# google-deepmind/mujoco_warp

Hardware: AMD Instinct MI355X
Metric: env-steps/sec (nworld x steps/s) for humanoid.xml at 8192 worlds, 1/2/4/8 GPUs (higher is better)
Workload: dtype f32; 1 GPU; humanoid.xml, nworld=8192 per GPU, CG solver, Euler, pyramidal, nconmax=24, njmax=64, key 0 + Halton/OU control noise (std 0.01, rate 0.1); nworld_per_gpu=8192, nworld_total=8192, parallelism=worlds sharded over 1 GPU(s), no data-path collective

## Files before the change

### include/mjhip.h

```cpp
#ifndef MJHIP_H
#define MJHIP_H

#ifdef __cplusplus
extern "C" {
#endif

#define MJH_OK 0
#define MJH_E_ARG -1
#define MJH_E_UNSUPPORTED -2
#define MJH_E_LAUNCH -3

#define MJH_STAGE_KINEMATICS 0
#define MJH_STAGE_COM_POS 1
#define MJH_STAGE_CRB 2
#define MJH_STAGE_FACTOR_M 3
#define MJH_STAGE_COLLISION 4
#define MJH_STAGE_MAKE_CONSTRAINT 5
#define MJH_STAGE_TRANSMISSION 6
#define MJH_STAGE_COM_VEL 7
#define MJH_STAGE_PASSIVE 8
#define MJH_STAGE_RNE 9
#define MJH_STAGE_FWD_VELOCITY 10
#define MJH_STAGE_FWD_ACTUATION 11
#define MJH_STAGE_FWD_ACCELERATION 12
// ... 209 lines not shown
  float* actuator_length; float* actuator_moment;
  float* actuator_velocity; float* cvel; float* cdof_dot;
  float* qfrc_spring; float* qfrc_damper; float* qfrc_gravcomp; float* qfrc_passive; float* qfrc_bias;
  float* cacc; float* cfrc_int; float* cfrc_ext;
  float* act_dot; float* actuator_force; float* qfrc_actuator; float* qfrc_smooth; float* qacc_smooth;
  float* qacc; float* qfrc_constraint; float* efc_Ma;
  int* solver_niter; int* ne; int* nf; int* nl; int* nefc; int* overflow;
  int* nacon; int* ncollision;
  float* contact_dist; float* contact_pos; float* contact_frame; float* contact_includemargin;
  float* contact_friction; float* contact_solref; float* contact_solreffriction; float* contact_solimp;
  int* contact_dim; int* contact_geom; int* contact_efc_address; int* contact_worldid; int* contact_type;
  int* contact_geomcollisionid;
  int* efc_type; int* efc_id; int* efc_state;
  float* efc_J; float* efc_pos; float* efc_margin; float* efc_D; float* efc_vel; float* efc_aref;
  float* efc_frictionloss; float* efc_force;
  int* ws_ncon;
  int* ws_conadr;
  int* ws_ncollision;
  float* ws_ccd;
  int* ws_tree_rowadr;
  int* ws_tree_rowmap;
  int* ws_isl_dofadr;
  int* ws_isl_dofmap;
  int* ws_isl_dofinv;
  int* ws_nisland;
  int* ws_isl_flags;
  int* ws_isl_list;
  int* ws_isl_count;
  int* ws_separable;
  float* sensordata;
  float* subtree_linvel; float* subtree_angmom;
  float* energy;
  int* tree_asleep;
  int* tree_awake;
  int* body_awake;
  int* body_awake_ind;
  int* dof_awake_ind;
  int* ntree_awake; int* nbody_awake; int* nv_awake;
  int* tree_island;
  int* nisland;
  float* ws_iacc;
  float* ws_pgsB;
  float* ws_sleep_J;
  float* ws_sleep_warm;
  int* ws_sleep_flag;
  int sleep_pass;
  int nvmax;
  int* ws_efc_con;
  int* ws_order;
  int* eq_active;
  float* ws_rk;
  float* history;
  float* ws_ctrl_delayed;
  float* ws_contact;
} MjhData;

int mjh_stage(const MjhModel* m, const MjhData* d, int stage, void* stream);

int mjh_step(const MjhModel* m, const MjhData* d, void* stream);
int mjh_forward(const MjhModel* m, const MjhData* d, void* stream);

int mjh_solve_m(const MjhModel* m, const MjhData* d, float* x, const float* y, void* stream);
int mjh_mul_m(const MjhModel* m, const MjhData* d, float* res, const float* vec, void* stream);
int mjh_qld_dense(const MjhModel* m, const MjhData* d, float* qld_dense, int stride, void* stream);
int mjh_contact_force(const MjhModel* m, const MjhData* d, const int* contact_ids, int n, int to_world_frame, float* force, void* stream);
int mjh_jac(const MjhModel* m, const MjhData* d, float* jacp, float* jacr, const float* point, const int* body, void* stream);
int mjh_rays(const MjhModel* m, const MjhData* d, const float* pnt, const float* vec, int pnt_nworld, int nray, const float* geomgroup,
             int flg_static, const int* bodyexclude, float* dist, int* geomid, float* normal, void* stream);
int mjh_efc_j_sparse(const MjhModel* m, const MjhData* d, int njmax_nnz, int* rownnz, int* rowadr, int* colind, float* values, void* stream);

#define MJH_SET_CONST_FIXED 1
#define MJH_SET_CONST_0 2
int mjh_set_const(const MjhModel* m, int nbatch, float* body_subtreemass, float* dof_invweight0, float* body_invweight0, float* stat_meaninertia, int what,
                  void* stream);

typedef struct MjhRender {
  int nworld;
  int ncam;
  int npixel;
  int ntile;
  int groupmask;
  const int* cam_bodyid;
  const float* cam_pos;
  const float* cam_quat;
  const int* cam_res;
  const int* cam_exclude;
  const int* depth_adr;
  const int* seg_adr;
  const int* tile;
  const float* ray;
  float* depth;
  int* seg;
  float* normal;
  float* cam_xpos;
  float* cam_xmat;
} MjhRender;
int mjh_render(const MjhModel* m, const MjhData* d, const MjhRender* rc, void* stream);
int mjh_camera_rays(const MjhModel* m, const MjhData* d, const MjhRender* rc, float* pnt, float* vec, void* stream);

int mjh_ctrl_noise(const MjhModel* m, const MjhData* d, const float* ctrl_center, int step, float noise_std,
                   float noise_rate, void* stream);

int mjh_history_read(const MjhModel* m, const MjhData* d, int is_sensor, int id, const float* time, int interp, float* result, int result_stride,
                     void* stream);
int mjh_history_init(const MjhModel* m, const MjhData* d, int is_sensor, int id, const float* times, const float* values, int values_stride,
                     const float* phase, void* stream);
// ... 24 lines not shown
```

### mujoco_warp_amd/csrc/host.hpp

```cpp
#pragma once
#include <hip/hip_runtime.h>

#include <algorithm>
#include <cstdio>
#include <cstdlib>
#include <cstring>
#include <mutex>
#include <type_traits>
#include <vector>

#include "../../include/mjhip.h"
#include "dev_common.hpp"

int mjh_fail(int code, const char* fmt, const char* a = "");
#define fail mjh_fail
#define HIPCHK(expr)                                                      \
  do {                                                                    \
    hipError_t e_ = (expr);                                               \
    if (e_ != hipSuccess) return fail(MJH_E_LAUNCH, #expr ": %s", hipGetErrorString(e_)); \
  } while (0)

static const int kLdsPerCU = 160 * 1024;

const char* mjh_knob(const char* name);
// ... 24 lines not shown
  }
}
template <typename F>
static inline int dispatch_nv4_64(int nv4, F&& f) {
  if (nv4 <= 9) return f(std::integral_constant<int, 9>{});
  if (nv4 <= 10) return f(std::integral_constant<int, 10>{});
  if (nv4 <= 12) return f(std::integral_constant<int, 12>{});
  if (nv4 <= 14) return f(std::integral_constant<int, 14>{});
  return f(std::integral_constant<int, 16>{});
}

#ifdef MJH_PHASE_CLOCK
#define MJH_DEFINE_PHASE_TICKS                                                                                                      \
  extern "C" __attribute__((visibility("default"))) int mjh_debug_phase_ticks(unsigned long long* out, int reset) {               \
    if (out) HIPCHK(hipMemcpyFromSymbol(out, HIP_SYMBOL(g_phase_ticks), sizeof(unsigned long long) * 64 * 8 * 16));                 \
    if (reset) {                                                                                                                    \
      static unsigned long long zeros[64 * 8 * 16] = {0};                                                                           \
      HIPCHK(hipMemcpyToSymbol(HIP_SYMBOL(g_phase_ticks), zeros, sizeof(zeros)));                                                   \
    }                                                                                                                               \
    return MJH_OK;                                                                                                                  \
  }
#else
#define MJH_DEFINE_PHASE_TICKS
#endif

int pick_block(size_t shared_bytes, size_t per_world_bytes, int G, size_t* lds_out, bool prefer_small_arg = false);

template <typename K>
static hipError_t set_lds(K kernel, size_t bytes) {
  if (bytes <= 64 * 1024) return hipSuccess;
  static std::mutex mu;
  static std::vector<std::pair<const void*, size_t>> done;
  const void* f = reinterpret_cast<const void*>(kernel);
  std::lock_guard<std::mutex> lock(mu);
  for (auto& p : done)
    if (p.first == f && p.second >= bytes) return hipSuccess;
  hipError_t e = hipFuncSetAttribute(f, hipFuncAttributeMaxDynamicSharedMemorySize, (int)bytes);
  if (e == hipSuccess) done.emplace_back(f, bytes);
  return e;
}

template <typename K>
static void debug_occupancy(const char* name, K kernel, int grid, int threads, size_t lds) {
  if (!KNOB_ONCE_FLAG("MJH_DEBUG_OCC")) return;
  int nb = -1;
  (void)hipOccupancyMaxActiveBlocksPerMultiprocessor(&nb, kernel, threads, lds);
  fprintf(stderr, "%-22s grid %5d x %3d threads, LDS %6zu B: %2d workgroups per CU = %4.1f wavefronts per SIMD, %.2f rounds on 256 CUs\n", name, grid,
          threads, lds, nb, nb * (threads / 64) / 4.0, nb > 0 ? grid / (256.0 * nb) : 0.0);
}

int launch_solve_32_cg(const MjhModel* m, const MjhData* d, int nr, bool with_factor, int fuse_euler, hipStream_t s, int lo, int hi);
int launch_solve_32_newton_ell_r1(const MjhModel* m, const MjhData* d, bool with_factor, int fuse_euler, hipStream_t s, int lo, int hi);
int launch_solve_cgw(const MjhModel* m, const MjhData* d, bool with_factor, int fuse_euler, hipStream_t s, int lo, int hi);
int launch_solve_32_cg_deferred(const MjhModel* m, const MjhData* d, int fuse_euler, hipStream_t s);
int launch_solve_cgp(const MjhModel* m, const MjhData* d, bool with_factor, int fuse_euler, hipStream_t s);
int launch_solve_32_newton(const MjhModel* m, const MjhData* d, int nr, bool with_factor, int fuse_euler, hipStream_t s, int lo, int hi);
int launch_solve_newton_mfma(const MjhModel* m, const MjhData* d, bool with_factor, int fuse_euler, hipStream_t s);
int launch_solve_64_cg(const MjhModel* m, const MjhData* d, int nr, bool with_factor, int fuse_euler, hipStream_t s, int lo, int hi);
int launch_solve_64_newton(const MjhModel* m, const MjhData* d, int nr, bool with_factor, int fuse_euler, hipStream_t s, int lo, int hi);
int launch_solve_32_cg_ell(const MjhModel* m, const MjhData* d, int nr, bool with_factor, int fuse_euler, hipStream_t s, int lo, int hi);
int launch_solve_32_newton_ell(const MjhModel* m, const MjhData* d, int nr, bool with_factor, int fuse_euler, hipStream_t s, int lo, int hi);
int launch_solve_64_cg_ell(const MjhModel* m, const MjhData* d, int nr, bool with_factor, int fuse_euler, hipStream_t s, int lo, int hi);
int launch_solve_64_newton_ell(const MjhModel* m, const MjhData* d, int nr, bool with_factor, int fuse_euler, hipStream_t s, int lo, int hi);
int launch_solve_tree_cg(const MjhModel* m, const MjhData* d, hipStream_t s, hipStream_t sr, hipStream_t sr2, hipStream_t sr3);
int launch_solve_tree_newton(const MjhModel* m, const MjhData* d, hipStream_t s, hipStream_t sr, hipStream_t sr2, hipStream_t sr3);
int launch_solve_tree_cg_ell(const MjhModel* m, const MjhData* d, hipStream_t s, hipStream_t sr, hipStream_t sr2, hipStream_t sr3);
int launch_solve_tree_newton_ell(const MjhModel* m, const MjhData* d, hipStream_t s, hipStream_t sr, hipStream_t sr2, hipStream_t sr3);
int launch_pgs(const MjhModel* m, const MjhData* d, hipStream_t s);
int launch_pgs_big(const MjhModel* m, const MjhData* d, hipStream_t s);
int launch_solve_big(const MjhModel* m, const MjhData* d, hipStream_t s, int nefc_lo = -1);
int launch_render(const MjhModel* m, const MjhData* d, const MjhRender* rc, hipStream_t s);
int launch_camera_rays(const MjhModel* m, const MjhData* d, const MjhRender* rc, float* pnt, float* vec, hipStream_t s);
int launch_sensor_contact(const MjhModel* m, const MjhData* d, hipStream_t s);
int launch_sensor_collision(const MjhModel* m, const MjhData* d, hipStream_t s);
int launch_transmission(const MjhModel* m, const MjhData* d, hipStream_t s);
int launch_vel_trn(const MjhModel* m, const MjhData* d, int first, int last, bool lanes64, hipStream_t s);
int launch_history_ctrl(const MjhModel* m, const MjhData* d, int insert, hipStream_t s);
int launch_history_sensor(const MjhModel* m, const MjhData* d, int stage, int insert, hipStream_t s);
```

### mujoco_warp_amd/csrc/mjhip.hip

```cpp
#include "host.hpp"

#include "contact_rec.hpp"
#ifdef MJH_CON_WINDOW
#undef CON_WINDOW
#define CON_WINDOW MJH_CON_WINDOW
#endif
#ifndef MJH_MID_WAVES
#define MJH_MID_WAVES 4
#endif

#include "collide.hpp"
#include "constraint.hpp"
#include "dev_common.hpp"
#include "integrate.hpp"
#include "implicit.hpp"
#include "sensor.hpp"
#include "sleep.hpp"
#include "smooth.hpp"
#include "support.hpp"

static thread_local char g_err[512] = "";
int mjh_fail(int code, const char* fmt, const char* a) {
  snprintf(g_err, sizeof(g_err), fmt, a);
  return code;
// ... 434 lines not shown
    const int inl_force = KNOB_ONCE_INT("MJH_NEWTON_RIDERS", -1);
    const bool inl = step && !instrumented && (inl_force >= 0 ? inl_force != 0 : m->nv <= 16) && plan_family(m, d, p.ell, 0) == FAM_NEWTON_MFMA;
    const bool side = p.newton && m->nv <= KNOB_ONCE_INT("MJH_SIDE_NV", 32) && !instrumented && !inl && side_ok && !KNOB_ONCE_FLAG("MJH_NO_SIDE");
    p.riders = inl || (m->solver == SOL_CG && m->nv <= 64) ? RIDE_SOLVER : side ? RIDE_SIDE : RIDE_INTEGRATOR;
    const bool fusable = step && m->na == 0 && p.riders != RIDE_INTEGRATOR && m->nv <= 64 &&
                         m->nsensor_acc == 0 &&
                         d->njmax <= 192;
    p.fuse_euler = !fusable ? 0
                   : (m->integrator == INT_EULER && (m->disableflags & (DSBL_EULERDAMP | DSBL_DAMPER)) != 0) ? 1
                   : (m->integrator == INT_IMPLICITFAST && !KNOB_ONCE_FLAG("MJH_NO_FUSE_IMPLICITFAST") && !m->act_velfeedback) ? 2 : 0;
  }
  p.family = plan_family(m, d, p.ell, p.fuse_euler);
  p.r1 = p.family == FAM_NEWTON32_ELL && d->njmax > 32 && KNOB_ONCE_INT("MJH_SOLVE_R1", 1) != 0;
  return p;
}
static int launch_solve_any(const MjhModel* m, const MjhData* d, const StepPlan& p, const Run& run) {
  const hipStream_t s = run.s;
  const int fe = p.fuse_euler, all = 0x7fffffff;
  const bool with_factor = p.riders == RIDE_SOLVER;
  const int top = d->njmax > 192 ? 192 : all;
  switch (p.family) {
    case FAM_UNSUPPORTED: return solve_supported(m, d);
    case FAM_PGS: return launch_pgs(m, d, s);
    case FAM_PGS_BIG: return launch_pgs_big(m, d, s);
    case FAM_BIG: return launch_solve_big(m, d, s);
    case FAM_TREE_BIG: {
      hipLaunchKernelGGL(k_isl_clear, dim3(1), dim3(64), 0, s, *d);
      hipLaunchKernelGGL(k_tree_rows, dim3(d->nworld), dim3(64), sizeof(int) * (size_t)(2 * std::max(d->njmax, 1) + 2 * m->ntree), s, *m, *d);
      Streams* aux = side_streams(run);
      if (aux && aux->n < MJH_NAUX) aux = nullptr;
      int naux = 0;
      if (aux) {
        hipStreamCaptureStatus cst = hipStreamCaptureStatusNone;
        naux = (hipStreamIsCapturing(s, &cst) == hipSuccess && cst == hipStreamCaptureStatusActive) ? MJH_NAUX : MJH_NAUX_EAGER;
        const int cap = KNOB_ONCE_INT("MJH_NAUX", -1);
        if (cap >= 2 && cap <= MJH_NAUX) naux = cap;
      }
      hipStream_t s1 = aux ? aux->stream[0] : s, s2 = aux ? aux->stream[1] : s, s3 = naux > 2 ? aux->stream[2] : s1, s4 = naux > 3 ? aux->stream[3] : s1;
      if (aux) {
        HIPCHK(hipEventRecord(aux->fork, s));
        for (int k = 0; k < naux; ++k) HIPCHK(hipStreamWaitEvent(aux->stream[k], aux->fork, 0));
      }
      int rc = (p.newton ? (p.ell ? launch_solve_tree_newton_ell : launch_solve_tree_newton) : (p.ell ? launch_solve_tree_cg_ell : launch_solve_tree_cg))(m, d, s, s1, s3, s4);
      if (!rc) rc = launch_solve_big(m, d, s2);
      if (aux) {
        for (int k = 0; k < naux; ++k) {
          HIPCHK(hipEventRecord(aux->join[k], aux->stream[k]));
          HIPCHK(hipStreamWaitEvent(s, aux->join[k], 0));
        }
      }
      return rc;
    }
    case FAM_NEWTON_MFMA: return launch_solve_newton_mfma(m, d, with_factor, fe, s);
    case FAM_CGP: {
      if (int rc = launch_solve_cgp(m, d, with_factor, fe, s)) return rc;
      return launch_solve_32_cg_deferred(m, d, fe, s);
    }
    case FAM_CGW:
    case FAM_PAIR:
    case FAM_CG32_ELL:
    case FAM_NEWTON32:
    case FAM_NEWTON32_ELL: {
      auto s32 = p.ell ? (p.newton ? launch_solve_32_newton_ell : launch_solve_32_cg_ell) : (p.newton ? launch_solve_32_newton : launch_solve_32_cg);
      const bool wide = p.family == FAM_CGW;
      int lo2 = -1;
      if (p.r1) {
        if (int rc = launch_solve_32_newton_ell_r1(m, d, false, fe, s, -1, 32)) return rc;
        lo2 = 32;
      }
      if (d->njmax <= 64) return wide ? launch_solve_cgw(m, d, with_factor, fe, s, -1, all) : s32(m, d, 2, with_factor, fe, s, lo2, all);
      if (int rc = wide ? launch_solve_cgw(m, d, false, fe, s, -1, 64) : s32(m, d, 2, false, fe, s, lo2, 64)) return rc;
      if (int rc = s32(m, d, 6, with_factor, fe, s, 64, top)) return rc;
      return d->njmax > 192 ? launch_solve_big(m, d, s, 192) : MJH_OK;
    }
    case FAM_CG64:
    case FAM_CG64_ELL:
    case FAM_NEWTON64:
    case FAM_NEWTON64_ELL: {
      auto s64 = p.ell ? (p.newton ? launch_solve_64_newton_ell : launch_solve_64_cg_ell) : (p.newton ? launch_solve_64_newton : launch_solve_64_cg);
      if (d->njmax <= 64) return s64(m, d, 1, with_factor, fe, s, -1, all);
      if (d->njmax <= 128) return s64(m, d, 2, with_factor, fe, s, -1, all);
      if (int rc = s64(m, d, 2, with_factor, fe, s, -1, 128)) return rc;
      if (int rc = s64(m, d, 3, false, fe, s, 128, top)) return rc;
      return d->njmax > 192 ? launch_solve_big(m, d, s, 192) : MJH_OK;
    }
  }
  return fail(MJH_E_ARG, "launch_solve_any: unknown solver family");
}
static int launch_solve(const MjhModel* m, const MjhData* d, const Run& run) { return launch_solve_any(m, d, plan_step(m, d, MJH_STAGE_SOLVE, run.instr != nullptr), run); }
static const char* solver_kernel_name(const MjhModel* m, const MjhData* d) { return kFamilyName[plan_step(m, d, MJH_STAGE_STEP, false).family]; }
static int launch_integrate_plus(const MjhModel* m, const MjhData* d, int mode, bool integrate, bool with_factor, hipStream_t s) {
  constexpr int G = 32;
  const IntLayout lay = int_layout(m->nv, m->nC);
  const FacLayout fl = fac_layout(m->nv, m->nC);
  const size_t ms_bytes = sizeof(int) * mstruct_ints(m->nv, m->nC);
  size_t lds = std::max(ms_bytes + sizeof(float) * std::max(lay.total, fl.total) * (256 / G), (size_t)2048);
  if (lds > (size_t)kLdsPerCU) return fail(MJH_E_UNSUPPORTED, "k_integrate: does not fit in LDS");
  HIPCHK(set_lds(k_integrate_plus<G>, lds));
  const int nb = (d->nworld + 256 / G - 1) / (256 / G);
  const int nint = integrate ? nb : 0, npub = with_factor ? nb : 0, nfac = with_factor ? nb : 0;
  if (nint + npub + nfac == 0) return MJH_OK;
  if (integrate && mode == 2) TRY(launch_implicit(m, d, s));
  debug_occupancy("k_integrate_plus", k_integrate_plus<G>, nint + npub + nfac, 256, lds);
  hipLaunchKernelGGL(k_integrate_plus<G>, dim3(nint + npub + nfac), dim3(256), lds, s, *m, *d, mode, nint, npub);
  return MJH_OK;
}
static void apply_noise(const MjhModel* m, const MjhData* d, Run& run) {
  const NoiseArgs noise = run.noise;
  run.noise.n = 0;
  if (noise.n == 0) return;
// ... 484 lines not shown
```

### mujoco_warp_amd/csrc/solve_cg32.hip

```cpp
#include "solve_tu.hpp"

int launch_solve_32_cg(const MjhModel* m, const MjhData* d, int nr, bool with_factor, int fuse_euler, hipStream_t s, int lo, int hi) {
  switch (nr) {
    case 2: return launch_solve_32<2, false>(m, d, with_factor, fuse_euler, s, lo, hi);
    case 6: return launch_solve_32<6, false>(m, d, with_factor, fuse_euler, s, lo, hi);
    default: return fail(MJH_E_ARG, "k_solve: unsupported rows per lane");
  }
}

int launch_solve_32_cg_deferred(const MjhModel* m, const MjhData* d, int fuse_euler, hipStream_t s) {
  return dispatch_nv4_32((m->nv + 3) / 4, [&](auto NV4) { return launch_solve_deferred_t<NV4(), 2, false, 32>(m, d, fuse_euler, s); });
}

MJH_DEFINE_PHASE_TICKS
```

### mujoco_warp_amd/csrc/solve_cgp.hip

```cpp
#include "host.hpp"

#include "contact_rec.hpp"
#include "smooth.hpp"
#include "solver_cgp.hpp"

#ifndef CGP_WAVES
#define CGP_WAVES 3
#endif
#define CGP_MAXT (256 * CGP_WAVES)
template <int NV4>
__global__ void __launch_bounds__(CGP_MAXT) __attribute__((amdgpu_waves_per_eu(CGP_WAVES, CGP_WAVES))) k_solve_cgp_plus(MjhModel m, MjhData d, int nsolve, int nfac, int fuse_euler, int pool_rows) {
  extern __shared__ __attribute__((aligned(16))) float smem[];
  const int wpb = blockDim.x / 32;
  if ((int)blockIdx.x < nsolve) solve_cgp_body<NV4>(m, d, smem, (int)blockIdx.x * wpb, wpb, pool_rows, fuse_euler);
  else {
    const int bi = (int)blockIdx.x - nsolve;
    if (bi < nfac) factor_smooth_body<32>(m, d, 0, smem, Blk{bi * wpb, wpb, (int)blockDim.x});
    else publish_body<32>(d, 1, reinterpret_cast<int*>(smem), Blk{(bi - nfac) * wpb, wpb, (int)blockDim.x}, m.nexplicit ? m.pair_solreffriction : nullptr);
  }
}
template <int NV4>
static int launch_cgp_t(const MjhModel* m, const MjhData* d, bool with_factor, int fuse_euler, hipStream_t s) {
  int threads = 128;
  if (const char* e = knob_str("MJH_CGP_THREADS")) threads = std::min(CGP_MAXT, std::max(64, (atoi(e) / 64) * 64));
  size_t lds = ((size_t)kLdsPerCU / (256 * CGP_WAVES / threads)) & ~(size_t)1023;
  if (const char* e = knob_str("MJH_CGP_LDS")) lds = (size_t)atoi(e);
  const int wpb = threads / 32;
  const int pool_rows = cgp_pool_rows<NV4>(lds, wpb);
  if (pool_rows < cgp_min_rows<NV4>(fuse_euler)) return fail(MJH_E_UNSUPPORTED, "k_solve_cgp: pool too small");
  const FacLayout fl = fac_layout(m->nv, m->nC);
  if (with_factor) lds = std::max(lds, sizeof(int) * mstruct_ints(m->nv, m->nC) + sizeof(float) * fl.total * wpb);
  if (lds > (size_t)kLdsPerCU) return fail(MJH_E_UNSUPPORTED, "k_solve_cgp: the workgroup does not fit in LDS");
  HIPCHK(set_lds(k_solve_cgp_plus<NV4>, lds));
  const int nsolve = (d->nworld + wpb - 1) / wpb, nfac = with_factor ? nsolve : 0;
  debug_occupancy("k_solve_cgp_plus", k_solve_cgp_plus<NV4>, nsolve + 2 * nfac, threads, lds);
  hipLaunchKernelGGL(k_solve_cgp_plus<NV4>, dim3(nsolve + 2 * nfac), dim3(threads), lds, s, *m, *d, nsolve, nfac, fuse_euler, pool_rows);
  return MJH_OK;
}
int launch_solve_cgp(const MjhModel* m, const MjhData* d, bool with_factor, int fuse_euler, hipStream_t s) {
  return dispatch_nv4_32((m->nv + 3) / 4, [&](auto NV4) { return launch_cgp_t<NV4()>(m, d, with_factor, fuse_euler, s); });
}

MJH_DEFINE_PHASE_TICKS
```

### mujoco_warp_amd/csrc/solve_tu.hpp

```cpp
#pragma once
#include "host.hpp"

#include "contact_rec.hpp"
#include "smooth.hpp"
#include "solver.hpp"

#ifndef MJH_N64_WAVES
#define MJH_N64_WAVES 1
#endif

template <int NV4, int NR, bool NEWTON, int SG, bool ELL = false>
__global__ void __launch_bounds__(256) __attribute__((amdgpu_waves_per_eu((!NEWTON && !ELL && SG == 32 && NR == 2) ? 3 : ((NEWTON && SG == 64 && MJH_N64_WAVES > 1) ? MJH_N64_WAVES : 1), 8))) k_solve_plus(MjhModel m, MjhData d, int nsolve, int nfac, int nefc_lo, int nefc_hi, int fuse_euler, int rider_at) {
  extern __shared__ __attribute__((aligned(16))) float smem[];
  const int wpb = blockDim.x / SG;
  const int bx = (int)blockIdx.x, nrider = NEWTON ? 0 : 2 * nfac;
  const int sb = bx < rider_at ? bx : bx - nrider;
  if (bx < rider_at || bx >= rider_at + nrider) solve_body<NV4, NR, NEWTON, SG, ELL>(m, d, smem, Blk{sb * wpb, wpb, (int)blockDim.x}, nefc_lo, nefc_hi, fuse_euler);
  else if (!NEWTON) {
    const int wf = blockDim.x / 32, bi = bx - rider_at;
    if (bi < nfac) factor_smooth_body<32>(m, d, 0, smem, Blk{bi * wf, wf, (int)blockDim.x});
    else publish_body<32>(d, 1, reinterpret_cast<int*>(smem), Blk{(bi - nfac) * wf, wf, (int)blockDim.x}, m.nexplicit ? m.pair_solreffriction : nullptr);
  }
}
template <int NV4, int NR, bool NEWTON, int SG, bool ELL = false>
static int launch_solve_t(const MjhModel* m, const MjhData* d, bool with_factor, int fuse_euler, hipStream_t s, int nefc_lo, int nefc_hi) {
  const SolveLayout lay = solve_layout<NV4, NR, SG, NEWTON, ELL>(std::min(d->njmax, nefc_hi));
  const FacLayout fl = fac_layout(m->nv, m->nC);
  const size_t ms_bytes = sizeof(int) * mstruct_ints(m->nv, m->nC);
  size_t lds;
  int threads = pick_block(0, sizeof(float) * lay.total, SG, &lds, true);
  if (!threads) return fail(MJH_E_UNSUPPORTED, "k_solve: njmax x nv does not fit in LDS");
  if (const char* e = knob_str("MJH_SOLVE_THREADS")) {
    threads = std::max(atoi(e), SG);
    lds = sizeof(float) * lay.total * (threads / SG);
  }
  const int wpb = threads / SG, wf = threads / 32;
  with_factor = with_factor && !NEWTON;
  if (with_factor) lds = std::max(lds, ms_bytes + sizeof(float) * fl.total * wf);
  HIPCHK(set_lds((k_solve_plus<NV4, NR, NEWTON, SG, ELL>), lds));
  const int nsolve = (d->nworld + wpb - 1) / wpb, nfac = with_factor ? (d->nworld + wf - 1) / wf : 0;
  debug_occupancy(NEWTON ? "k_solve_plus<newton>" : "k_solve_plus<cg>", k_solve_plus<NV4, NR, NEWTON, SG, ELL>, nsolve + 2 * nfac, threads, lds);
  const int rider_pct = KNOB_ONCE_INT("MJH_RIDER_AT", 100);
  const int rider_at = std::min(nsolve, (int)((long long)nsolve * std::max(rider_pct, 0) / 100));
  hipLaunchKernelGGL((k_solve_plus<NV4, NR, NEWTON, SG, ELL>), dim3(nsolve + 2 * nfac), dim3(threads), lds, s, *m, *d, nsolve, nfac, nefc_lo, nefc_hi, fuse_euler, rider_at);
  return MJH_OK;
}
template <int NV4, int NR, bool NEWTON, int SG, bool ELL = false>
__global__ void __launch_bounds__(256) k_solve_deferred(MjhModel m, MjhData d, int fuse_euler) {
  extern __shared__ __attribute__((aligned(16))) float smem[];
  const int wpb = blockDim.x / SG;
  const int lig = threadIdx.x & (SG - 1), gid = (int)blockIdx.x * wpb + (int)threadIdx.x / SG;
  for (int c0 = gid * SG; c0 < d.nworld; c0 += (int)gridDim.x * wpb * SG) {
    unsigned long long todo = gballot<SG>(c0 + lig < d.nworld && d.solver_niter[c0 + lig] == -1);
    while (todo) {
      const int bq = __ffsll((long long)todo) - 1;
      todo &= todo - 1ull;
      solve_body<NV4, NR, NEWTON, SG, ELL>(m, d, smem, Blk{0, wpb, (int)blockDim.x}, -1, 0x7fffffff, fuse_euler, 0, 0x7fffffff, c0 + bq);
      gsync();
    }
  }
}
template <int NV4, int NR, bool NEWTON, int SG, bool ELL = false>
static int launch_solve_deferred_t(const MjhModel* m, const MjhData* d, int fuse_euler, hipStream_t s) {
  const SolveLayout lay = solve_layout<NV4, NR, SG, NEWTON, ELL>(d->njmax);
  size_t lds;
  const int threads = pick_block(0, sizeof(float) * lay.total, SG, &lds, true);
  if (!threads) return fail(MJH_E_UNSUPPORTED, "k_solve_deferred: njmax x nv does not fit in LDS");
  HIPCHK(set_lds((k_solve_deferred<NV4, NR, NEWTON, SG, ELL>), lds));
  const int wpb = threads / SG;
  hipLaunchKernelGGL((k_solve_deferred<NV4, NR, NEWTON, SG, ELL>), dim3(std::max(1, (d->nworld + wpb * SG - 1) / (wpb * SG))), dim3(threads), lds, s, *m, *d, fuse_euler);
  return MJH_OK;
}
template <int NR, bool NEWTON, bool ELL = false>
static int launch_solve_32(const MjhModel* m, const MjhData* d, bool wf, int fe, hipStream_t s, int lo, int hi) {
  return dispatch_nv4_32((m->nv + 3) / 4, [&](auto NV4) { return launch_solve_t<NV4(), NR, NEWTON, 32, ELL>(m, d, wf, fe, s, lo, hi); });
}
template <int NR, bool NEWTON, bool ELL = false>
static int launch_solve_64(const MjhModel* m, const MjhData* d, bool wf, int fe, hipStream_t s, int lo, int hi) {
  return dispatch_nv4_64((m->nv + 3) / 4, [&](auto NV4) { return launch_solve_t<NV4(), NR, NEWTON, 64, ELL>(m, d, wf, fe, s, lo, hi); });
}
```

### mujoco_warp_amd/csrc/solver.hpp

```cpp
#pragma once
#include "dev_common.hpp"
#include "smooth.hpp"

template <int G>
DEV float bcastg(float v, int k) {
  const int a = __builtin_amdgcn_readlane(__float_as_int(v), k);
  if (G == 64) return __int_as_float(a);
  const int b = __builtin_amdgcn_readlane(__float_as_int(v), k + 32);
  return __int_as_float((threadIdx.x & 32) ? b : a);
}
template <int G>
DEV float gsumg(float v) {
  v = dpp_add_f<0x111, 0xf, 0xf>(v);
  v = dpp_add_f<0x112, 0xf, 0xf>(v);
  v = dpp_add_f<0x114, 0xf, 0xf>(v);
  v = dpp_add_f<0x118, 0xf, 0xf>(v);
  v = dpp_add_f<0x142, 0xa, 0xf>(v);
  if (G == 64) {
    v = dpp_add_f<0x143, 0xc, 0xf>(v);
    return bcastg<64>(v, 63);
  }
  return __int_as_float(__builtin_amdgcn_ds_swizzle(__float_as_int(v), 0x3E0));
}
template <int G, int N>
// ... 589 lines not shown
    gsync();
    float P[4][4], Pi[4][4];
#pragma unroll
    for (int p = 0; p < 4; ++p) {
      const float4 v = *reinterpret_cast<const float4*>(pb + p * NVR + k);
      P[p][0] = v.x; P[p][1] = v.y; P[p][2] = v.z; P[p][3] = v.w;
#pragma unroll
      for (int e = 0; e < 4; ++e) Pi[p][e] = p == e ? 1.0f : 0.0f;
    }
#pragma unroll
    for (int j = 0; j < 4; ++j) {
      const float ip = 1.0f / P[j][j];
#pragma unroll
      for (int e = 0; e < 4; ++e) {
        P[j][e] *= ip;
        Pi[j][e] *= ip;
      }
#pragma unroll
      for (int r = 0; r < 4; ++r)
        if (r != j) {
          const float f = P[r][j];
#pragma unroll
          for (int e = 0; e < 4; ++e) {
            P[r][e] -= f * P[j][e];
            Pi[r][e] -= f * Pi[j][e];
          }
        }
    }
    const bool inb = q >= 0 && q < 4;
    float F[4];
#pragma unroll
    for (int p = 0; p < 4; ++p) {
      const float out = s[k] * Pi[0][p] + s[k + 1] * Pi[1][p] + s[k + 2] * Pi[2][p] + s[k + 3] * Pi[3][p];
      const float own = (q == p ? 1.0f : 0.0f) - (q == 0 ? Pi[0][p] : (q == 1 ? Pi[1][p] : (q == 2 ? Pi[2][p] : Pi[3][p])));
      F[p] = inb ? own : out;
    }
#pragma unroll
    for (int c4 = 0; c4 < NVR / 4; ++c4) {
      if (c4 == kb) continue;
      const float4 r0 = *reinterpret_cast<const float4*>(pb + 4 * c4), r1 = *reinterpret_cast<const float4*>(pb + NVR + 4 * c4),
                   r2 = *reinterpret_cast<const float4*>(pb + 2 * NVR + 4 * c4), r3 = *reinterpret_cast<const float4*>(pb + 3 * NVR + 4 * c4);
      s[4 * c4] -= F[0] * r0.x + F[1] * r1.x + F[2] * r2.x + F[3] * r3.x;
      s[4 * c4 + 1] -= F[0] * r0.y + F[1] * r1.y + F[2] * r2.y + F[3] * r3.y;
      s[4 * c4 + 2] -= F[0] * r0.z + F[1] * r1.z + F[2] * r2.z + F[3] * r3.z;
      s[4 * c4 + 3] -= F[0] * r0.w + F[1] * r1.w + F[2] * r2.w + F[3] * r3.w;
    }
#pragma unroll
    for (int e = 0; e < 4; ++e) s[k + e] = (q == e ? 1.0f : 0.0f) - F[e];
  }
}

template <int NV4, int NR, bool NEWTON, int G, bool ELL = false, bool TREE = false>
DEV void solve_body(const MjhModel& m, const MjhData& d, float* smem, const Blk& b, int nefc_lo = -1, int nefc_hi = 0x7fffffff,
                    int fuse_euler = 0, int nv_lo = 0, int nv_hi = 0x7fffffff, int w_direct = -1) {
  if ((int)threadIdx.x >= b.nthreads) return;
  constexpr int NVR = 4 * NV4;
  constexpr int JS = (NV4 & 1) ? NVR : NVR + 4;
  const int nv_all = m.nv, nC = m.nC, njmax = d.njmax, nvp = d.nv_pad;
  const SolveLayout lay = solve_layout<NV4, NR, G, NEWTON, ELL, TREE>(TREE ? njmax : min(njmax, nefc_hi));
  const int lig = threadIdx.x & (G - 1), gib = threadIdx.x / G;
  const int slot = b.w0 + gib;
  if (TREE && gib >= b.nw) return;
  if (w_direct < 0 && slot >= (TREE ? d.nworld * m.ntree : d.nworld)) return;
  const int w = TREE ? slot / m.ntree : (w_direct >= 0 ? w_direct : d.ws_order[slot]);
  const int tree = TREE ? slot - w * m.ntree : 0;
  if (TREE && (!d.ws_separable[w] || tree >= d.ws_nisland[w])) return;
  const int* dadr = TREE ? d.ws_isl_dofadr + (size_t)w * (m.ntree + 1) + tree : nullptr;
  const int nv = TREE ? dadr[1] - dadr[0] : nv_all;
  if (TREE && (nv <= nv_lo || nv > nv_hi)) return;
  const int* dmap = TREE ? d.ws_isl_dofmap + (size_t)w * nv_all + dadr[0] : nullptr;
  const int* dinv = TREE ? d.ws_isl_dofinv + (size_t)w * nv_all : nullptr;
  const int* rmap = TREE ? d.ws_tree_rowmap + (size_t)w * njmax + d.ws_tree_rowadr[(size_t)w * (m.ntree + 1) + tree] : nullptr;
  auto R = [&](int r) __attribute__((always_inline)) { return TREE ? rmap[r] : r; };
  float* S = smem + (size_t)gib * lay.total;
  float *Jl = S + lay.J, *eforce = S + lay.force, *eda = S + lay.da, *bsearch = S + lay.bsearch, *bgrad = S + lay.bgrad, *col = S + lay.col;
  constexpr int GR = G * NR;
  float *exu = S + lay.ex, *exv = exu + GR, *exq0 = exv + GR, *exq1 = exq0 + GR, *exq2 = exq1 + GR, *exs = exq2 + GR;
  float* econe = S + lay.cone;
  int* einfo = reinterpret_cast<int*>(S + lay.cone) + 6 * GR;

  const int nefc_all = TREE ? d.ws_tree_rowadr[(size_t)w * (m.ntree + 1) + tree + 1] - d.ws_tree_rowadr[(size_t)w * (m.ntree + 1) + tree]
                            : min(d.nefc[w], njmax);
  if (nefc_all <= nefc_lo || nefc_all > nefc_hi) return;
  const int nefc = min(nefc_all, G * NR);
  const int ne = TREE ? 0 : d.ne[w], nf = TREE ? 0 : d.nf[w];
  const size_t vo = TREE ? (size_t)w * nv_all + (lig < nv ? dmap[lig] : 0) - lig : (size_t)w * nv_all, eo = (size_t)w * njmax;
  float* flds = S + lay.fl;
  bool has_fl = nf > 0;
  if (TREE) {
    bool any = false;
    for (int r = lig; r < G * NR; r += G) {
      const bool fr = r < nefc && (d.efc_type[eo + rmap[r]] == CT_FRICTION_DOF || d.efc_type[eo + rmap[r]] == CT_FRICTION_TENDON);
      flds[r] = fr ? d.efc_frictionloss[eo + rmap[r]] : 0.0f;
      any |= fr;
    }
    has_fl = gballot<G>(any) != 0ull;
    gsync();
  }
  const float* floss = TREE ? flds : d.efc_frictionloss + eo;
  const bool active = lig < nv;
  const int ligr = lig < NVR ? lig : NVR - 1;

  PhaseClock pc(5, lig);
  float mrow[NVR];
  if (!TREE) {
    const float* Mg = d.M + (size_t)w * nC;
    const int nv4r = (nv_all + 3) >> 2;
    const int4* tab = reinterpret_cast<const int4*>(m.M_dense) + (size_t)(active ? lig : 0) * nv4r;
    int idx[NVR];
#pragma unroll
    for (int c4 = 0; c4 < NV4; ++c4) {
      const int4 t4 = c4 < nv4r ? tab[c4] : make_int4(-1, -1, -1, -1);
      idx[4 * c4] = t4.x; idx[4 * c4 + 1] = t4.y; idx[4 * c4 + 2] = t4.z; idx[4 * c4 + 3] = t4.w;
    }
#pragma unroll
    for (int c = 0; c < NVR; ++c) {
      const float v = Mg[idx[c] < 0 ? 0 : idx[c]];
      mrow[c] = active ? (idx[c] < 0 ? 0.0f : v) : (c == lig ? 1.0f : 0.0f);
    }
  } else {
    for (int idx = lig; idx < NVR * JS; idx += G) Jl[idx] = 0.0f;
    gsync();
    const float* Mg = d.M + (size_t)w * nC;
    for (int i = lig; i < nv; i += G) {
      const int gi = TREE ? dmap[i] : i;
      const int start = m.M_rowadr[gi], n = m.M_rownnz[gi];
      for (int a = 0; a < n; ++a) {
// ... 566 lines not shown
```

### mujoco_warp_amd/csrc/solver_cgp.hpp

```cpp
#pragma once
#include <type_traits>
#include "solver.hpp"
#include "solver_cgw.hpp"

#ifndef MJH_CGP_HOIST
#define MJH_CGP_HOIST 1
#endif
#define CGP_HEAD 32
#define CGP_WORLD 136
template <int NV4>
__host__ __device__ inline int cgp_pool_rows(size_t lds_bytes, int wpb) {
  constexpr int NVR = 4 * NV4, JS = (NV4 & 1) ? NVR : NVR + 4;
  const int words = (int)(lds_bytes / sizeof(float)) - CGP_HEAD - CGP_WORLD * wpb;
  return words <= 0 ? 0 : ((words / JS) & ~3);
}
template <int NV4>
__host__ __device__ inline int cgp_min_rows(int fuse_euler) {
  constexpr int NVR = 4 * NV4, JS = (NV4 & 1) ? NVR : NVR + 4;
  const int words = fuse_euler == 2 ? (6 * 32 + 12 * NV4 + 4 + 32) : (8 * NVR > 32 ? 8 * NVR : 32);
  return (((words + JS - 1) / JS) + 3) & ~3;
}

template <int CTRL>
DEV float qperm(float v) {
// ... 135 lines not shown
  {
    const float* Mg = d.M + (size_t)w * nC;
#pragma unroll
    for (int c = 0; c < NVR; ++c) {
      const float v = Mg[idx[c] < 0 ? 0 : idx[c]];
      mrow[c] = active ? (idx[c] < 0 ? 0.0f : v) : (c == lig ? 1.0f : 0.0f);
    }
  }
  const float fs = active ? d.qfrc_smooth[vo + lig] : 0.0f;
  const float qwarm = active ? d.qacc_warmstart[vo + lig] : 0.0f;

  int np = 0, nq = 0, need = 0;
  bool defer = false;
  if (valid) {
    npf = min(npf, nefc);
    bool is6[2];
#pragma unroll
    for (int k = 0; k < 2; ++k) {
      const int r = lig + G * k;
      is6[k] = r >= npf && r < nefc && ty[k] == CT_CONTACT_PYRAMIDAL;
    }
    const unsigned m0 = (unsigned)gballot<G>(is6[0]), m1 = (unsigned)gballot<G>(is6[1]);
    const int n60 = __popc(m0), n6 = n60 + __popc(m1);
    const unsigned below = (1u << lig) - 1u;
#pragma unroll
    for (int k = 0; k < 2; ++k) {
      const int r = lig + G * k;
      const int c6 = k == 0 ? __popc(m0 & below) : n60 + __popc(m1 & below);
      if (r < nefc && r < 64) slotR[is6[k] ? c6 : n6 + r - c6] = r;
      fbT[r] = 0.0f;
    }
    nq = n6 >> 2;
    np = nefc - n6;
    defer = nf > 0 || (n6 & 3) != 0 || nefc > 64;
    need = max((np + 3 * nq + 15) & ~15, cgp_min_rows<NV4>(fuse_euler));
  }
  if (lig == 0 && gib < CGP_HEAD) cnt[gib] = (valid && !defer) ? need : 0;
  __syncthreads();
  int base = 0;
  {
    int acc = 0;
    for (int j = 0; j < nwb; ++j) {
      const int c = cnt[j];
      const bool fits = acc + c <= pool_rows;
      if (j == gib) {
        base = acc;
        if (!fits) defer = true;
      }
      acc += fits ? c : 0;
    }
  }
  if (!valid) return;
  if (defer) {
    if (lig == 0) d.solver_niter[w] = -1;
    return;
  }
  float* Jl = pool + (size_t)base * JS;
  const int nb = np + 3 * nq, nb16 = (nb + 15) & ~15;

  PhaseClock pc(5, lig);
  pc.mark(0);
  const bool warm = !(m.disableflags & DSBL_WARMSTART);
  auto mul_row = [&](const float (&row)[NVR], BV x) __attribute__((always_inline)) {
    float s[2] = {0.0f, 0.0f};
    dpp_fence(x);
    fmac_seq<0, NVR, NA>(s, row, x.a);
    if constexpr (NBX > 0) fmac_seq<NA, NVR, NBX>(s, row, x.b);
    return active ? s[0] + s[1] : 0.0f;
  };
  float h[NVR];
  invert_rows_b4s<NVR, G>(mrow, h, Jl, lig);
  float qs = mul_row(h, bcast_prep(fs));
  {
    const float res = fs - mul_row(mrow, bcast_prep(qs));
    qs += mul_row(h, bcast_prep(active ? res : 0.0f));
  }
  if (active) d.qacc_smooth[vo + lig] = qs;
  float q = active ? (nefc > 0 && warm ? qwarm : qs) : 0.0f;
  pc.mark(1);
  float Ma = mul_row(mrow, bcast_prep(q));
  if (nefc == 0) {
    if (active) {
      d.qacc[vo + lig] = q;
      d.qfrc_constraint[vo + lig] = 0.0f;
      d.efc_Ma[vo + lig] = Ma;
    }
    if (lig == 0) d.solver_niter[w] = 0;
    if (fuse_euler) {
      float qi = q;
      gsync();
      if (fuse_euler == 2) qi = impfast_acc<NV4, G>(m, d, w, lig, active, mrow, Ma, Jl);
      euler_advance<G>(m, d, w, lig, active, qi, Jl + (fuse_euler == 2 ? 6 * G + 12 * NV4 + 4 : 0), q);
    }
    return;
  }

  float rD[NR], rja[NR], rjv[NR];
  int rkind[NR];
  int jro[NR];
  int fbo[NR];
  bool isq[NR];
  int rer[NR];
  const int qd = lig & 3;
#pragma unroll
  for (int k = 0; k < NR; ++k) {
    const int s = lig + G * k;
    const bool has = s < nefc;
// ... 269 lines not shown
```

### mujoco_warp_amd/types.py

```python

import dataclasses
import enum

import numpy as np

from .device import DeviceArray


class BroadphaseType(enum.IntEnum):
  NXN = 0
  SAP_TILE = 1
  SAP_SEGMENTED = 2


class BroadphaseFilter(enum.IntFlag):
  PLANE = 1 << 0
  SPHERE = 1 << 1
  AABB = 1 << 2
  OBB = 1 << 3


class OverflowType(enum.IntFlag):
  NEFC = 1 << 0
  NJMAX_NNZ = 1 << 1
# ... 617 lines not shown
  subtree_com: DeviceArray = _arr(('nworld', 'nbody', 3), "float32")
  cinert: DeviceArray = _arr(('nworld', 'nbody', 10), "float32")
  cdof: DeviceArray = _arr(('nworld', 'nv', 6), "float32")
  crb: DeviceArray = _arr(('nworld', 'nbody', 10), "float32")
  M: DeviceArray = _arr(('nworld', 'nC'), "float32")
  qLD: DeviceArray = _arr(('nworld', 'nC'), "float32")
  qLDiagInv: DeviceArray = _arr(('nworld', 'nv'), "float32")
  actuator_length: DeviceArray = _arr(('nworld', 'nu'), "float32")
  actuator_moment: DeviceArray = _arr_own(('nworld', 'nJmom'), "float32")
  moment_rownnz: DeviceArray = _arr(('nworld', 'nu'), "int32")
  moment_rowadr: DeviceArray = _arr(('nworld', 'nu'), "int32")
  moment_colind: DeviceArray = _arr_own(('nworld', 'nJmom'), "int32")
  actuator_velocity: DeviceArray = _arr(('nworld', 'nu'), "float32")
  cvel: DeviceArray = _arr(('nworld', 'nbody', 6), "float32")
  cdof_dot: DeviceArray = _arr(('nworld', 'nv', 6), "float32")
  qfrc_spring: DeviceArray = _arr(('nworld', 'nv'), "float32")
  qfrc_damper: DeviceArray = _arr(('nworld', 'nv'), "float32")
  qfrc_gravcomp: DeviceArray = _arr(('nworld', 'nv'), "float32")
  qfrc_passive: DeviceArray = _arr(('nworld', 'nv'), "float32")
  qfrc_bias: DeviceArray = _arr(('nworld', 'nv'), "float32")
  cacc: DeviceArray = _arr(('nworld', 'nbody', 6), "float32")
  cfrc_int: DeviceArray = _arr(('nworld', 'nbody', 6), "float32")
  act_dot: DeviceArray = _arr(('nworld', 'na'), "float32")
  actuator_force: DeviceArray = _arr(('nworld', 'nu'), "float32")
  qfrc_actuator: DeviceArray = _arr(('nworld', 'nv'), "float32")
  qfrc_smooth: DeviceArray = _arr(('nworld', 'nv'), "float32")
  qacc_smooth: DeviceArray = _arr(('nworld', 'nv'), "float32")
  qacc: DeviceArray = _arr(('nworld', 'nv'), "float32")
  qfrc_constraint: DeviceArray = _arr(('nworld', 'nv'), "float32")
  solver_niter: DeviceArray = _arr(('nworld',), "int32")
  ne: DeviceArray = _arr(('nworld',), "int32")
  nf: DeviceArray = _arr(('nworld',), "int32")
  nl: DeviceArray = _arr(('nworld',), "int32")
  nefc: DeviceArray = _arr(('nworld',), "int32")
  overflow: DeviceArray = _arr(('nworld',), "int32")
  nacon: DeviceArray = _arr((1,), "int32")
  ncollision: DeviceArray = _arr((1,), "int32")
  ws_ncon: DeviceArray = _arr(('nworld',), "int32")
  ws_conadr: DeviceArray = _arr(('nworld',), "int32")
  ws_ncollision: DeviceArray = _arr(('nworld',), "int32")
  ws_efc_con: DeviceArray = _arr(('nworld', 'njmax'), "int32")
  ws_tree_rowadr: DeviceArray = _arr(('nworld', 'ntreeadr'), "int32")
  ws_tree_rowmap: DeviceArray = _arr(('nworld', 'ntreerow'), "int32")
  ws_isl_dofadr: DeviceArray = _arr(('nworld', 'ntreeadr'), "int32")
  ws_isl_dofmap: DeviceArray = _arr(('nworld', 'ntreedof'), "int32")
  ws_isl_dofinv: DeviceArray = _arr(('nworld', 'ntreedof'), "int32")
  ws_nisland: DeviceArray = _arr(('nworld',), "int32")
  ws_isl_flags: DeviceArray = _arr(('nworld',), "int32")
  ws_isl_list: DeviceArray = _arr((3, 'ntreeworld'), "int32")
  ws_isl_count: DeviceArray = _arr((4,), "int32")
  ws_separable: DeviceArray = _arr(('nworld',), "int32")
  ws_ccd: DeviceArray = _arr(('nccdworld', 'nccdword', 32), "float32")
  ws_order: DeviceArray = _arr(('nworld',), "int32")
  sensordata: DeviceArray = _arr(('nworld', 'nsensordata'), "float32")
  energy: DeviceArray = _arr(('nworld', 2), "float32")
  subtree_linvel: DeviceArray = _arr(('nworld', 'nbody', 3), "float32")
  subtree_angmom: DeviceArray = _arr(('nworld', 'nbody', 3), "float32")
  cfrc_ext: DeviceArray = _arr(('nworld', 'nbody', 6), "float32")
  tree_asleep: DeviceArray = _arr(('nworld', 'ntree'), "int32")
  tree_awake: DeviceArray = _arr(('nworld', 'ntree'), "int32")
  body_awake: DeviceArray = _arr(('nworld', 'nbody'), "int32")
  body_awake_ind: DeviceArray = _arr(('nworld', 'nbody'), "int32")
  dof_awake_ind: DeviceArray = _arr(('nworld', 'nv'), "int32")
  ntree_awake: DeviceArray = _arr(('nworld',), "int32")
  nbody_awake: DeviceArray = _arr(('nworld',), "int32")
  nv_awake: DeviceArray = _arr(('nworld',), "int32")
  tree_island: DeviceArray = _arr(('nworld', 'ntree'), "int32")
  nisland: DeviceArray = _arr(('nworld',), "int32")
  ws_iacc: DeviceArray = _arr(('nimpworld', 'nv'), "float32")
  ws_pgsB: DeviceArray = _arr(('npgsworld', 'njmax_pad', 'nv_pad'), "float32")
  ws_sleep_J: DeviceArray = _arr(('nsleepworld', 'njmax_pad', 'nv_pad'), "float32")
  ws_sleep_warm: DeviceArray = _arr(('nsleepworld', 'nv'), "float32")
  ws_sleep_flag: DeviceArray = _arr(('nworld',), "int32")
  sleep_pass: int = 0
  nimpworld: int = 0
  npgsworld: int = 0
  nvmax: int = 0
  nsleepworld: int = 0
  eq_active: DeviceArray = _arr(('nworld', 'neq'), "int32")
  ws_rk: DeviceArray = _arr(('nworld', 'nq+3*nv+2*na'), "float32")
  ws_contact: DeviceArray = _arr(('nworld', 'concap', 32), "float32")
  history: DeviceArray = _arr_own(('nworld', 'nhistory'), "float32")
  ws_ctrl_delayed: DeviceArray = _arr(('nworld', 'nu'), "float32")
  nworld: int = 0
  nconmax: int = 0
  naconmax: int = 0
  njmax: int = 0
  njmax_pad: int = 0
  nv_pad: int = 0
  nmaxpyramid: int = 0
  nccdworld: int = 0
  nccdword: int = 0
  world_offset: int = 0
  concap: int = 0
  nccdhand: int = 0
  njmax_nnz: int = 0
```

Baseline: 27.87 million env-steps/s.

## Fold deferred CG fallback solve into last-finishing block of CGP kernel

Removes the separate k_solve_deferred launch after the CGP solver. Worlds whose constraint rows do not fit the LDS pool now increment a global counter; the last wave to finish, chosen by an atomic ticket, solves those deferred worlds inside the same kernel, reloading the kernel arguments from the kernarg segment. This saves a kernel launch and its full grid scan of solver_niter. In exchange, deferred worlds run serially in a single workgroup, the kernel's LDS request grows to the fallback layout size, and a new 8-byte control word must be allocated and zeroed.

```diff
diff --git a/include/mjhip.h b/include/mjhip.h
--- a/include/mjhip.h
+++ b/include/mjhip.h
@@ -285,6 +285,7 @@
   float* ws_rk;
   float* history;
   float* ws_ctrl_delayed;
+  int* ws_cgp_ctl;
   float* ws_contact;
 } MjhData;
 
diff --git a/mujoco_warp_amd/csrc/host.hpp b/mujoco_warp_amd/csrc/host.hpp
--- a/mujoco_warp_amd/csrc/host.hpp
+++ b/mujoco_warp_amd/csrc/host.hpp
@@ -100,7 +100,6 @@
 int launch_solve_32_cg(const MjhModel* m, const MjhData* d, int nr, bool with_factor, int fuse_euler, hipStream_t s, int lo, int hi);
 int launch_solve_32_newton_ell_r1(const MjhModel* m, const MjhData* d, bool with_factor, int fuse_euler, hipStream_t s, int lo, int hi);
 int launch_solve_cgw(const MjhModel* m, const MjhData* d, bool with_factor, int fuse_euler, hipStream_t s, int lo, int hi);
-int launch_solve_32_cg_deferred(const MjhModel* m, const MjhData* d, int fuse_euler, hipStream_t s);
 int launch_solve_cgp(const MjhModel* m, const MjhData* d, bool with_factor, int fuse_euler, hipStream_t s);
 int launch_solve_32_newton(const MjhModel* m, const MjhData* d, int nr, bool with_factor, int fuse_euler, hipStream_t s, int lo, int hi);
 int launch_solve_newton_mfma(const MjhModel* m, const MjhData* d, bool with_factor, int fuse_euler, hipStream_t s);
diff --git a/mujoco_warp_amd/csrc/mjhip.hip b/mujoco_warp_amd/csrc/mjhip.hip
--- a/mujoco_warp_amd/csrc/mjhip.hip
+++ b/mujoco_warp_amd/csrc/mjhip.hip
@@ -510,10 +510,7 @@
       return rc;
     }
     case FAM_NEWTON_MFMA: return launch_solve_newton_mfma(m, d, with_factor, fe, s);
-    case FAM_CGP: {
-      if (int rc = launch_solve_cgp(m, d, with_factor, fe, s)) return rc;
-      return launch_solve_32_cg_deferred(m, d, fe, s);
-    }
+    case FAM_CGP: return launch_solve_cgp(m, d, with_factor, fe, s);
     case FAM_CGW:
     case FAM_PAIR:
     case FAM_CG32_ELL:
diff --git a/mujoco_warp_amd/csrc/solve_cg32.hip b/mujoco_warp_amd/csrc/solve_cg32.hip
--- a/mujoco_warp_amd/csrc/solve_cg32.hip
+++ b/mujoco_warp_amd/csrc/solve_cg32.hip
@@ -8,8 +8,4 @@
   }
 }
 
-int launch_solve_32_cg_deferred(const MjhModel* m, const MjhData* d, int fuse_euler, hipStream_t s) {
-  return dispatch_nv4_32((m->nv + 3) / 4, [&](auto NV4) { return launch_solve_deferred_t<NV4(), 2, false, 32>(m, d, fuse_euler, s); });
-}
-
 MJH_DEFINE_PHASE_TICKS
diff --git a/mujoco_warp_amd/csrc/solve_cgp.hip b/mujoco_warp_amd/csrc/solve_cgp.hip
--- a/mujoco_warp_amd/csrc/solve_cgp.hip
+++ b/mujoco_warp_amd/csrc/solve_cgp.hip
@@ -8,12 +8,54 @@
 #define CGP_WAVES 3
 #endif
 #define CGP_MAXT (256 * CGP_WAVES)
+typedef __attribute__((address_space(3))) float CgpLdsFloat;
+typedef const __attribute__((address_space(4))) char CgpKernargByte;
+DEV void cgp_ctl_reset(const MjhData& d) {
+  if ((threadIdx.x & 63) == 0) __hip_atomic_store(reinterpret_cast<unsigned long long*>(d.ws_cgp_ctl), 0ull, __ATOMIC_RELAXED, __HIP_MEMORY_SCOPE_AGENT);
+}
+template <int NV4>
+__device__ __attribute__((noinline, noreturn)) void cgp_fallback_worlds(CgpKernargByte* ka_arg, CgpLdsFloat* lds, int fuse_euler) {
+  static_assert(alignof(MjhModel) <= 8 && alignof(MjhData) <= 8, "kernel-argument layout of k_solve_cgp_plus");
+  const unsigned long long kau = (unsigned long long)ka_arg;
+  const unsigned klo = (unsigned)__builtin_amdgcn_readfirstlane((int)(unsigned)kau), khi = (unsigned)__builtin_amdgcn_readfirstlane((int)(unsigned)(kau >> 32));
+  CgpKernargByte* ka = (CgpKernargByte*)(((unsigned long long)khi << 32) | klo);
+  const MjhModel& m = *(const MjhModel*)ka;
+  const MjhData& d = *(const MjhData*)(ka + ((sizeof(MjhModel) + 7) & ~(size_t)7));
+  float* smem = (float*)lds;
+  const int lig = threadIdx.x & 31, wave = (int)threadIdx.x >> 6;
+  for (int c0 = (int)(threadIdx.x & 32); c0 < d.nworld; c0 += 64) {
+    unsigned long long todo = gballot<32>(c0 + lig < d.nworld && d.solver_niter[c0 + lig] == -1);
+    while (todo) {
+      const int bq = __ffsll((long long)todo) - 1;
+      todo &= todo - 1ull;
+      solve_body<NV4, 2, false, 32, false>(m, d, smem, Blk{0, (int)blockDim.x / 32, (int)blockDim.x}, -1, 0x7fffffff, fuse_euler, 0, 0x7fffffff, c0 + bq, 2 * wave);
+      gsync();
+    }
+  }
+  cgp_ctl_reset(d);
+  __builtin_amdgcn_endpgm();
+}
+template <int NV4>
+DEV void cgp_fallback_role(const MjhData& d, float* smem, int nsolve, int fuse_euler) {
+  unsigned long long t = 0ull;
+  if ((threadIdx.x & 63) == 0) t = atomicAdd(reinterpret_cast<unsigned long long*>(d.ws_cgp_ctl), 1ull);
+  const int ticket = __builtin_amdgcn_readlane((int)(unsigned)t, 0), nflag = __builtin_amdgcn_readlane((int)(unsigned)(t >> 32), 0);
+  if (ticket != nsolve * (int)(blockDim.x >> 6) - 1) return;
+  if (nflag > 0) {
+    __threadfence();
+    asm volatile("s_waitcnt vmcnt(0)" ::: "memory");
+    cgp_fallback_worlds<NV4>((CgpKernargByte*)__builtin_amdgcn_kernarg_segment_ptr(), (CgpLdsFloat*)smem, fuse_euler);
+  }
+  cgp_ctl_reset(d);
+}
 template <int NV4>
 __global__ void __launch_bounds__(CGP_MAXT) __attribute__((amdgpu_waves_per_eu(CGP_WAVES, CGP_WAVES))) k_solve_cgp_plus(MjhModel m, MjhData d, int nsolve, int nfac, int fuse_euler, int pool_rows) {
   extern __shared__ __attribute__((aligned(16))) float smem[];
   const int wpb = blockDim.x / 32;
-  if ((int)blockIdx.x < nsolve) solve_cgp_body<NV4>(m, d, smem, (int)blockIdx.x * wpb, wpb, pool_rows, fuse_euler);
-  else {
+  if ((int)blockIdx.x < nsolve) {
+    solve_cgp_body<NV4>(m, d, smem, (int)blockIdx.x * wpb, wpb, pool_rows, fuse_euler);
+    cgp_fallback_role<NV4>(d, smem, nsolve, fuse_euler);
+  } else {
     const int bi = (int)blockIdx.x - nsolve;
     if (bi < nfac) factor_smooth_body<32>(m, d, 0, smem, Blk{bi * wpb, wpb, (int)blockDim.x});
     else publish_body<32>(d, 1, reinterpret_cast<int*>(smem), Blk{(bi - nfac) * wpb, wpb, (int)blockDim.x}, m.nexplicit ? m.pair_solreffriction : nullptr);
@@ -28,6 +70,8 @@
   const int wpb = threads / 32;
   const int pool_rows = cgp_pool_rows<NV4>(lds, wpb);
   if (pool_rows < cgp_min_rows<NV4>(fuse_euler)) return fail(MJH_E_UNSUPPORTED, "k_solve_cgp: pool too small");
+  if (!d->ws_cgp_ctl || ((uintptr_t)d->ws_cgp_ctl & 7)) return fail(MJH_E_ARG, "Data.ws_cgp_ctl missing or not 8-byte aligned (two zeroed ints: allocate Data with make_data/put_data)");
+  lds = std::max(lds, 2 * sizeof(float) * (size_t)solve_layout<NV4, 2, 32, false, false>(d->njmax).total);
   const FacLayout fl = fac_layout(m->nv, m->nC);
   if (with_factor) lds = std::max(lds, sizeof(int) * mstruct_ints(m->nv, m->nC) + sizeof(float) * fl.total * wpb);
   if (lds > (size_t)kLdsPerCU) return fail(MJH_E_UNSUPPORTED, "k_solve_cgp: the workgroup does not fit in LDS");
diff --git a/mujoco_warp_amd/csrc/solve_tu.hpp b/mujoco_warp_amd/csrc/solve_tu.hpp
--- a/mujoco_warp_amd/csrc/solve_tu.hpp
+++ b/mujoco_warp_amd/csrc/solve_tu.hpp
@@ -45,32 +45,6 @@
   hipLaunchKernelGGL((k_solve_plus<NV4, NR, NEWTON, SG, ELL>), dim3(nsolve + 2 * nfac), dim3(threads), lds, s, *m, *d, nsolve, nfac, nefc_lo, nefc_hi, fuse_euler, rider_at);
   return MJH_OK;
 }
-template <int NV4, int NR, bool NEWTON, int SG, bool ELL = false>
-__global__ void __launch_bounds__(256) k_solve_deferred(MjhModel m, MjhData d, int fuse_euler) {
-  extern __shared__ __attribute__((aligned(16))) float smem[];
-  const int wpb = blockDim.x / SG;
-  const int lig = threadIdx.x & (SG - 1), gid = (int)blockIdx.x * wpb + (int)threadIdx.x / SG;
-  for (int c0 = gid * SG; c0 < d.nworld; c0 += (int)gridDim.x * wpb * SG) {
-    unsigned long long todo = gballot<SG>(c0 + lig < d.nworld && d.solver_niter[c0 + lig] == -1);
-    while (todo) {
-      const int bq = __ffsll((long long)todo) - 1;
-      todo &= todo - 1ull;
-      solve_body<NV4, NR, NEWTON, SG, ELL>(m, d, smem, Blk{0, wpb, (int)blockDim.x}, -1, 0x7fffffff, fuse_euler, 0, 0x7fffffff, c0 + bq);
-      gsync();
-    }
-  }
-}
-template <int NV4, int NR, bool NEWTON, int SG, bool ELL = false>
-static int launch_solve_deferred_t(const MjhModel* m, const MjhData* d, int fuse_euler, hipStream_t s) {
-  const SolveLayout lay = solve_layout<NV4, NR, SG, NEWTON, ELL>(d->njmax);
-  size_t lds;
-  const int threads = pick_block(0, sizeof(float) * lay.total, SG, &lds, true);
-  if (!threads) return fail(MJH_E_UNSUPPORTED, "k_solve_deferred: njmax x nv does not fit in LDS");
-  HIPCHK(set_lds((k_solve_deferred<NV4, NR, NEWTON, SG, ELL>), lds));
-  const int wpb = threads / SG;
-  hipLaunchKernelGGL((k_solve_deferred<NV4, NR, NEWTON, SG, ELL>), dim3(std::max(1, (d->nworld + wpb * SG - 1) / (wpb * SG))), dim3(threads), lds, s, *m, *d, fuse_euler);
-  return MJH_OK;
-}
 template <int NR, bool NEWTON, bool ELL = false>
 static int launch_solve_32(const MjhModel* m, const MjhData* d, bool wf, int fe, hipStream_t s, int lo, int hi) {
   return dispatch_nv4_32((m->nv + 3) / 4, [&](auto NV4) { return launch_solve_t<NV4(), NR, NEWTON, 32, ELL>(m, d, wf, fe, s, lo, hi); });
diff --git a/mujoco_warp_amd/csrc/solver.hpp b/mujoco_warp_amd/csrc/solver.hpp
--- a/mujoco_warp_amd/csrc/solver.hpp
+++ b/mujoco_warp_amd/csrc/solver.hpp
@@ -665,7 +665,7 @@
 
 template <int NV4, int NR, bool NEWTON, int G, bool ELL = false, bool TREE = false>
 DEV void solve_body(const MjhModel& m, const MjhData& d, float* smem, const Blk& b, int nefc_lo = -1, int nefc_hi = 0x7fffffff,
-                    int fuse_euler = 0, int nv_lo = 0, int nv_hi = 0x7fffffff, int w_direct = -1) {
+                    int fuse_euler = 0, int nv_lo = 0, int nv_hi = 0x7fffffff, int w_direct = -1, int gib0 = 0) {
   if ((int)threadIdx.x >= b.nthreads) return;
   constexpr int NVR = 4 * NV4;
   constexpr int JS = (NV4 & 1) ? NVR : NVR + 4;
@@ -685,7 +685,7 @@
   const int* dinv = TREE ? d.ws_isl_dofinv + (size_t)w * nv_all : nullptr;
   const int* rmap = TREE ? d.ws_tree_rowmap + (size_t)w * njmax + d.ws_tree_rowadr[(size_t)w * (m.ntree + 1) + tree] : nullptr;
   auto R = [&](int r) __attribute__((always_inline)) { return TREE ? rmap[r] : r; };
-  float* S = smem + (size_t)gib * lay.total;
+  float* S = smem + (size_t)(gib - gib0) * lay.total;
   float *Jl = S + lay.J, *eforce = S + lay.force, *eda = S + lay.da, *bsearch = S + lay.bsearch, *bgrad = S + lay.bgrad, *col = S + lay.col;
   constexpr int GR = G * NR;
   float *exu = S + lay.ex, *exv = exu + GR, *exq0 = exv + GR, *exq1 = exq0 + GR, *exq2 = exq1 + GR, *exs = exq2 + GR;
diff --git a/mujoco_warp_amd/csrc/solver_cgp.hpp b/mujoco_warp_amd/csrc/solver_cgp.hpp
--- a/mujoco_warp_amd/csrc/solver_cgp.hpp
+++ b/mujoco_warp_amd/csrc/solver_cgp.hpp
@@ -211,7 +211,12 @@
   }
   if (!valid) return;
   if (defer) {
-    if (lig == 0) d.solver_niter[w] = -1;
+    if (lig == 0) {
+      d.solver_niter[w] = -1;
+      atomicAdd(reinterpret_cast<unsigned long long*>(d.ws_cgp_ctl), 1ull << 32);
+    }
+    __threadfence();
+    asm volatile("s_waitcnt vmcnt(0)" ::: "memory");
     return;
   }
   float* Jl = pool + (size_t)base * JS;
diff --git a/mujoco_warp_amd/types.py b/mujoco_warp_amd/types.py
--- a/mujoco_warp_amd/types.py
+++ b/mujoco_warp_amd/types.py
@@ -693,6 +693,7 @@
   ws_separable: DeviceArray = _arr(('nworld',), "int32")
   ws_ccd: DeviceArray = _arr(('nccdworld', 'nccdword', 32), "float32")
   ws_order: DeviceArray = _arr(('nworld',), "int32")
+  ws_cgp_ctl: DeviceArray = _arr((2,), "int32")
   sensordata: DeviceArray = _arr(('nworld', 'nsensordata'), "float32")
   energy: DeviceArray = _arr(('nworld', 2), "float32")
   subtree_linvel: DeviceArray = _arr(('nworld', 'nbody', 3), "float32")
```

After: 28.02 million env-steps/s, median of 6. About the same (+0.5%).
